# jscanvic/Scale-Equivariant-Imaging

Hardware: AMD Instinct MI355X
Metric: training images/sec (256x256 crops), proposed-loss deblur (higher is better)
Workload: dtype bf16; 1 GPU; BASELINE configs[1]: deblurring Gaussian_R2 noise=5, proposed loss (SURE + scale-EI), 256x256 pairs cropped to 48 in Loss.forward, ConvolutionalModel hidden=32 scales=5; parameters=645063043, batch_per_gpu=32, global_batch=32, parallelism=dp1

## Files before the change

include/sei_hip.h:

```cpp
#ifndef SEI_HIP_H
#define SEI_HIP_H

#include <stddef.h>
#include <stdint.h>

#ifdef __cplusplus
extern "C" {
#endif

#define SEI_OK 0
#define SEI_ERR_BAD_ARG 10001
#define SEI_ERR_TOO_LARGE 10002


#define SEI_ABI_VERSION 12
int sei_abi_version(void);
int sei_build_target(char *name, int n);

int sei_event_create(void **event);
int sei_event_destroy(void *event);
int sei_event_record_external(void *event, void *stream);
int sei_stream_wait_event(void *stream, void *event);

int sei_graph_node_counts(void *graph, int *kernel_nodes, int *all_nodes);
// ... 301 lines not shown
                         float *D32, uint16_t *D16, int M, int N, int epilogue, const float *bias, void *stream);
int sei_gemm_bf16nt_conv_unpad(const uint16_t *Ap, int cin_pad, const int *row_off9, const uint16_t *B, int ldb, float *y,
                               const float *res, int Bimg, int H, int W, int N, const float *bias, int act, void *stream);

int sei_adam_fused(float *param, const void *grad, int grad_is_bf16, float *exp_avg, float *exp_avg_sq,
                   size_t n, float lr, float beta1, float beta2, float eps, float weight_decay, int step,
                   float grad_scale, uint16_t *param_bf16, void *stream);

int sei_gemm_bf16nt_dw2_adam(const uint16_t *A1, const uint16_t *A2, int lda, const uint16_t *B1, const uint16_t *B2,
                             int ldb, float *param, float *exp_avg, float *exp_avg_sq, uint16_t *param_bf16,
                             const float *hyper, int M, int N, int K1, int K2, void *stream);
int sei_gemm_bf16nt_dw2_adam_ex(const uint16_t *A1, const uint16_t *A2, int lda, const uint16_t *B1, const uint16_t *B2,
                                int ldb, float *param, float *exp_avg, float *exp_avg_sq, uint16_t *param_bf16,
                                const float *hyper, int M, int N, int K1, int K2, int tile, void *stream);
size_t sei_gemm_bf16nt_dw2_adam_plan(int M, int N, int K1, int K2, int tile);
int sei_adam_scalars(float lr, float beta1, float beta2, float eps, float weight_decay, int step, float *out6_host,
                     void *stream);
int sei_adam_scalars_to_device(float lr, float beta1, float beta2, float eps, float weight_decay, int step,
                               float *dev6, void *stream);

size_t sei_sgd_partials(size_t lo, size_t hi, int grid_cap);
int sei_sgd_fused(float *param, const float *grad, const float *anchor, const float *coef64, size_t lo, size_t hi,
                  float lr, float grad_scale, uint16_t *param_bf16, double *partials, int grid_cap, void *stream);
int sei_sgd_penalty_finish(const double *partials, size_t count, float *penalty, void *stream);

size_t sei_adam_anchor_partials(size_t lo, size_t hi, int grid_cap);
int sei_adam_anchor_fused(float *param, const float *grad, float *exp_avg, float *exp_avg_sq, const float *anchor,
                          const float *coef64, size_t lo, size_t hi, float lr, float beta1, float beta2, float eps,
                          float weight_decay, int step, float grad_scale, uint16_t *param_bf16, double *partials,
                          int grid_cap, void *stream);
// ... 128 lines not shown
```

scale-equivariant-imaging_amd/_native.py:

```python
import ctypes
import os

import torch

_HERE = os.path.dirname(os.path.abspath(__file__))
LIB_PATH = os.environ.get("SEI_HIP_LIBRARY") or os.path.join(_HERE, "libsei_hip.so")

SEI_REDUCE_BLOCKS = 256

_c = ctypes
_P, _I, _F, _Z, _L = _c.c_void_p, _c.c_int, _c.c_float, _c.c_size_t, _c.c_longlong

SIGNATURES = {
    "sei_abi_version": [],
    "sei_event_create": [_P],
    "sei_event_destroy": [_P],
    "sei_event_record_external": [_P, _P],
    "sei_stream_wait_event": [_P, _P],
    "sei_graph_node_counts": [_P, _P, _P],
    "sei_build_target": [_c.c_char_p, _I],
    "sei_blur_sep_circ": [_P, _P, _P, _P, _I, _I, _I, _I, _I, _I, _P],
    "sei_blur_dense_circ": [_P, _P, _P, _I, _I, _I, _I, _I, _I, _P],
    "sei_blur_dense_pad": [_P, _P, _P, _I, _I, _I, _I, _I, _I, _I, _P, _P],
    "sei_circ_filter_sep": [_P, _P, _P, _P, _I, _I, _I, _P],
# ... 61 lines not shown
    "sei_gelu_f32": [_P, _P, _Z, _P],
    "sei_mul_dgelu_f32": [_P, _P, _Z, _P],
    "sei_cast_transpose_bf16": [_P, _I, _P, _P, _I, _I, _I, _P, _P],
    "sei_cast_bf16_colsum_weighted": [_P, _P, _P, _P, _I, _I, _P],
    "sei_cast_bf16_colsum_parts": [_P, _P, _P, _P, _I, _I, _P],
    "sei_gemm_bf16nt": [_P, _I, _I, _P, _I, _I, _P, _P, _I, _I, _I, _I, _P, _P, _P, _P, _P],
    "sei_gemm_bf16nt_colsum": [_P, _I, _I, _P, _I, _I, _P, _I, _I, _I, _I, _P, _P, _P],
    "sei_gemm_bf16nt_ws": [_P, _I, _I, _P, _I, _I, _P, _P, _I, _I, _I, _I, _P, _P, _P, _P, _P, _P, _Z, _I, _I, _I, _P],
    "sei_fold_many": [_P, _I, _P],
    "sei_transpose_bf16_many": [_P, _I, _P],
    "sei_gemm_bf16nt_dw2": [_P, _P, _I, _P, _P, _I, _P, _I, _I, _I, _I, _I, _P],
    "sei_gemm_bf16nt_ex": [_P, _I, _I, _P, _I, _I, _P, _P, _I, _I, _I, _I, _P, _P, _P, _P, _I, _I, _P],
    "sei_gemm_bf16nt_dw2_ex": [_P, _P, _I, _P, _P, _I, _P, _I, _I, _I, _I, _I, _I, _P],
    "sei_gemm_bf16nt_dw2_adam": [_P, _P, _I, _P, _P, _I, _P, _P, _P, _P, _P, _I, _I, _I, _I, _P],
    "sei_gemm_bf16nt_dw2_adam_ex": [_P, _P, _I, _P, _P, _I, _P, _P, _P, _P, _P, _I, _I, _I, _I, _I, _P],
    "sei_gemm_bf16nt_dw2_bf16out": [_P, _P, _I, _P, _P, _I, _P, _I, _I, _I, _I, _P],
    "sei_gemm_bf16nt_dw2_taps": [_P, _P, _I, _P, _P, _I, _P, _I, _I, _I, _I, _I, _I, _P, _L, _P],
    "sei_sepmap2": [_P, _P, _I, _I, _I, _I, _I, _I, _P, _P, _P, _P, _P, _Z, _P],
    "sei_sepmap2_big_pack": [_P, _P, _P, _P, _P, _I, _I, _I, _I, _P],
    "sei_sepmap2_big": [_P, _P, _I, _I, _I, _I, _I, _I, _P, _P, _P],
    "sei_sepmap2_packed": [_P, _P, _I, _I, _I, _I, _I, _I, _P, _P, _P, _Z, _P],
    "sei_sepmap2_bf16": [_P, _P, _I, _I, _I, _I, _I, _I, _P, _P],
    "sei_sepmap2_bf16_pack": [_P, _P, _P, _P, _P, _I, _I, _I, _I, _P],
    "sei_sepmap2_small": [_P, _P, _I, _I, _I, _I, _I, _I, _I, _P, _P, _P, _P, _P],
    "sei_sepmap2_bf16_out16": [_P, _P, _I, _I, _I, _I, _I, _I, _P, _P],
    "sei_colsum_f32": [_P, _P, _Z, _I, _P],
    "sei_colsum_weighted_f32": [_P, _P, _P, _Z, _I, _P],
    "sei_mlp_fused_fwd": [_P, _P, _P, _P, _P, _P, _F, _P, _I, _I, _P],
    "sei_mlp_fused_bwd": [_P, _P, _P, _P, _P, _P, _P, _P, _P, _P, _I, _I, _P],
    "sei_swin_attn_fwd": [_P, _P, _P, _I, _I, _I, _I, _I, _I, _F, _P],
# ... 62 lines not shown
    _fields_ = [("Y1", _P), ("Y2", _P), ("X1", _P), ("X2", _P), ("ldy", _I), ("ldx", _I), ("y0", _I), ("x0", _I),
                ("D", _P), ("ldd", _I)]


TOKGRAD_MAX_BLOCKS = 16


class DwStreamJob(_c.Structure):
    _fields_ = [("Y1", _P), ("Y2", _P), ("X1", _P), ("X2", _P), ("ldy", _I), ("ldx", _I), ("Mo", _I), ("Ni", _I),
                ("D", _P), ("ldd", _I), ("reserved", _I), ("K1", _L), ("K2", _L), ("gbias", _P)]


DWSTREAM_MAX_JOBS = 64


class FoldJob(_c.Structure):
    _fields_ = [("a", _P), ("b", _P), ("c", _P), ("ncol", _I), ("split", _I), ("kind", _I), ("nseg", _I),
                ("part", _P * 3), ("groups", _I * 3), ("reserved", _I)]


FOLD_SPLIT, FOLD_DWCONV7, FOLD_MAX_JOBS = 0, 1, 48


class TransposeJob(_c.Structure):
    _fields_ = [("src", _P), ("dst", _P), ("R", _I), ("C", _I)]


TRANSPOSE_MAX_JOBS = 16

CG_STATE_WORDS, CG_DONE, CG_ITERATIONS = 8, 3, 4
# ... 20 lines not shown
    "sei_sepmap2_big_work_elems": [_I, _I, _I, _I, _I, _I],
    "sei_swin_partials_floats": [_I],
    "sei_tokgrad_bf16_eligible": [_I, _I, _I, _I, _L, _L],
    "sei_dwstream_bf16_eligible": [_I, _I, _I, _I, _L, _L],
    "sei_mlp_fused_eligible": [_L, _I],
    "sei_rowgemm_bf16_eligible": [_L, _I, _I, _I, _I],
    "sei_rowgemm_lnbwd_bf16_eligible": [_L, _I, _I],
    "sei_rowgemm_lnbwd_work_floats": [_I],
    "sei_ln_bwd_part_offset": [_Z, _I],
    "sei_ln_bwd_part_count": [_Z, _I],
    "sei_rowgemm_dgelu_bf16_eligible": [_L, _I, _I],
    "sei_rowgemm_ln_bf16_eligible": [_L, _I, _I],
    "sei_gemm_bf16nt_plan": [_I, _I, _I, _I, _I, _I, _I, _I],
    "sei_gemm_bf16nt_plan_ws": [_I, _I, _I, _I, _I, _I, _I, _I, _Z],
    "sei_gemm_bf16nt_dw2_adam_plan": [_I, _I, _I, _I, _I],
    "sei_conv3x3_bwd_weight_parts_count": [_I, _I, _I, _I, _I, _I, _I],
    "sei_sepmap2_small_eligible": [_I, _I, _I, _I, _I, _I],
    "sei_cast_bf16_colsum_parts_count": [_I, _I],
    "sei_sgd_partials": [_Z, _Z, _I],
    "sei_adam_anchor_partials": [_Z, _Z, _I],
    "sei_drunet_work_bytes": [_I, _I, _I],
    "sei_cg_partials": [_Z],
    "sei_dps_partials": [_I, _Z],
    "sei_bm3d_ref_blocks": [_I, _I, _I],
    "sei_adm_gn_part_floats": [_I, _I],
}
ABI_VERSION = 12


class NativeLibraryError(RuntimeError):
# ... 33 lines not shown
    else:
        code = lib().sei_gemm_bf16nt_plan(int(a_rmajor), int(b_rmajor), int(out_f32), int(out_bf16), M, Nn, K, epilogue)
    if code == 0:
        raise NativeLibraryError("sei_gemm_bf16nt_plan: arguments sei_gemm_bf16nt would refuse")
    plan = {1: "nt", 2: "pq"}[code >> 48], (code >> 32) & 0xFFFF, (code >> 16) & 0xFFFF, code & 0x7FFF
    return plan + (bool(code & 0x8000),) if ws_bytes else plan


def adam_gemm_plan(M, Nn, K1, K2, tile=0):
    code = lib().sei_gemm_bf16nt_dw2_adam_plan(M, Nn, K1, K2, tile)
    if code == 0:
        raise NativeLibraryError("sei_gemm_bf16nt_dw2_adam_plan: arguments sei_gemm_bf16nt_dw2_adam_ex would refuse")
    return {1: "nt", 2: "pq"}[code >> 48], (code >> 32) & 0xFFFF, (code >> 16) & 0xFFFF, code & 0x7FFF


def stream():
    return torch.cuda.current_stream().cuda_stream


def check_tensor(t, name="tensor", dtype=torch.float32):
    if not isinstance(t, torch.Tensor):
        raise TypeError(f"{name}: expected a torch.Tensor, got {type(t).__name__}")
    if not t.is_cuda:
        raise NativeLibraryError(
            f"{name} is on {t.device}: this build runs on MI355X only (HIP kernels, no CPU path); "
            "use the CPU oracle under oracle/ for host-side checks")
    if t.dtype != dtype:
        raise TypeError(f"{name}: expected {dtype}, got {t.dtype}")
    if not t.is_contiguous():
        raise ValueError(f"{name}: expected a contiguous tensor")
# ... 93 lines not shown
```

scale-equivariant-imaging_amd/csrc/gemm_bf16nt.hip:

```cpp
#include "rm_image.h"

namespace {

constexpr int BK = 64;
constexpr int ROW_BYTES = 128;
constexpr int NWAVES = 8, NT = 512;

__device__ __attribute__((aligned(16))) unsigned short g_zero_chunk[8] = {0, 0, 0, 0, 0, 0, 0, 0};

struct NtArgs {
    const unsigned short *A = nullptr, *B = nullptr;
    float *D32 = nullptr;
    unsigned short *D16 = nullptr;
    int M = 0, N = 0, K = 0, lda = 0, ldb = 0;
    int epilogue = 0;
    const float *bias = nullptr, *R1 = nullptr, *R2 = nullptr;
    unsigned short *D2_16 = nullptr;
    int splitk = 1, k_per_split = 0;
    int tiles_m = 0, tiles_n = 0;
    int tiles_per_xcd = 0, band = 0;
    const unsigned short *A2 = nullptr, *B2 = nullptr;
    int k_seg = 0;
    int force_tile = 0, force_band = 0;
    float *colsum = nullptr;
    unsigned long long *plan = nullptr;
    int conv_cin = 0;
    int conv_off[9] = {};
    float *adam_p = nullptr, *adam_m = nullptr, *adam_v = nullptr;
    unsigned short *adam_p16 = nullptr;
    const float *adam_h = nullptr;
    int batch = 1;
    int batch_row[9] = {};
    long long batch_ld = 0;
    int unpad_H = 0, unpad_W = 0, unpad_act = 0;
    float *ws_slab = nullptr;
    unsigned *ws_cnt = nullptr;
    void *ws = nullptr;
    size_t ws_bytes = 0;
    int force_splitk = 0;
};

__device__ __forceinline__ float4 nt_load4(const float *p) {
    const f32x4 v = __builtin_nontemporal_load(reinterpret_cast<const f32x4 *>(p));
    return make_float4(v.x, v.y, v.z, v.w);
}
__device__ __forceinline__ void nt_store4(float *p, const float4 v) {
    f32x4 t;
    t.x = v.x; t.y = v.y; t.z = v.z; t.w = v.w;
    __builtin_nontemporal_store(t, reinterpret_cast<f32x4 *>(p));
}


template <int ROWS>
__device__ __forceinline__ void stage_piece(const unsigned short *__restrict__ G, int ld, int row0, int row_lim,
// ... 65 lines not shown
    static_assert(!BRM || BN % 128 == 0, "a reduction-major B tile is BN/128 images of 64 k-rows x 128 columns");
    constexpr int KS = stage_rows<TN, ARM, BRM, NSTAGE>();
    constexpr int A_BYTES = BM * ROW_BYTES * KS / BK;
    constexpr int IMG = 256 * KS;
    constexpr int STAGE = (BM + BN) * ROW_BYTES * KS / BK;
    __shared__ __attribute__((aligned(1024))) char smem[NSTAGE * STAGE];

    const int lane = threadIdx.x & 63;
    const int wave = __builtin_amdgcn_readfirstlane(threadIdx.x >> 6);
    const int wm = wave / WN, wn = wave % WN;
    const int li = lane & 31, lh = lane >> 5;

    int bid = blockIdx.x;
    const unsigned short *Bp = g.B, *B2p = g.B2;
    float *D32p = g.D32;
    if constexpr (ROWEPI == 3) {
        const int per = gridDim.x / g.batch, bt = bid / per;
        bid -= bt * per;
        const ptrdiff_t shift = (ptrdiff_t)g.batch_row[bt] * g.ldb;
        Bp += shift;
        B2p += shift;
        D32p += (size_t)bt * g.batch_ld;
    }
    int zs, ord;
    if (g.tiles_per_xcd == 0) {
        const int ntile = g.tiles_m * g.tiles_n;
        zs = bid / ntile;
        ord = bid - zs * ntile;
    } else {
        const int per_split = 8 * g.tiles_per_xcd;
        zs = bid / per_split;
        bid -= zs * per_split;
        ord = (bid & 7) * g.tiles_per_xcd + (bid >> 3);
        if ((bid >> 3) >= g.tiles_per_xcd || ord >= g.tiles_m * g.tiles_n) return;
    }
    int tm_i, tn_i;
    {
        const int band_tiles = g.tiles_m * g.band;
        const int b = ord / band_tiles, r = ord - b * band_tiles;
        const int width = min(g.band, g.tiles_n - b * g.band);
        tm_i = r / width;
        tn_i = b * g.band + (r - tm_i * width);
    }
    const int m0 = tm_i * BM, n0 = tn_i * BN;
    const int M = g.M, N = g.N, K = g.K;
    const int k_begin = zs * g.k_per_split;
    const int k_end = min(K, k_begin + g.k_per_split);

    f32x16 acc[TM][TN];
#pragma unroll
    for (int i = 0; i < TM; ++i)
#pragma unroll
        for (int j = 0; j < TN; ++j)
#pragma unroll
            for (int r = 0; r < 16; ++r) acc[i][j][r] = 0.f;

    constexpr bool PREFETCH_AUX = false;
    const int epi = g.epilogue;
    const bool lead = zs == 0;
    const bool split = g.splitk > 1;
    const float *aux1p = nullptr, *aux2p = nullptr;
    if (epi == SEI_EPI_BIAS_RES && (!split || lead)) { aux1p = g.R1; aux2p = g.R2; }
// ... 25 lines not shown
#pragma unroll
                for (int j = 0; j < TN; ++j)
#pragma unroll
                    for (int r = 0; r < 16; ++r) a1[i][j][r] = a2[i][j][r] = 0.f;
        }
    }

    constexpr int NPA = ARM ? 2 * KS / BK : (BM + 63) / 64, NPB = (BN / 64) * KS / BK;
    static_assert(BN % 64 == 0, "whole pieces per wave");
    unsigned off_a[NPA], off_b[NPB];
#pragma unroll
    for (int e = 0; e < NPA; ++e) {
        const int q = wave + NWAVES * e;
        if constexpr (ARM) {
            const int row = 4 * q + (lane >> 4), ch = (lane & 15) ^ swz_rmajor(row);
            off_a[e] = (unsigned)row * (unsigned)g.lda * 2u + 2u * (unsigned)min(8 * ch, M - 8 - m0);
        } else {
            const int row = 8 * q + (lane >> 3), c = (lane & 7) ^ ((row >> 1) & 7);
            off_a[e] = (unsigned)min(row, M - 1 - m0) * (unsigned)g.lda * 2u + 16u * c;
        }
    }
#pragma unroll
    for (int e = 0; e < NPB; ++e) {
        const int q = wave + NWAVES * e;
        if constexpr (BRM) {
            constexpr int PPI = KS / 4;
            const int im = q / PPI, qq = q % PPI;
            const int row = 4 * qq + (lane >> 4), ch = (lane & 15) ^ swz_rmajor(row);
            off_b[e] = (unsigned)row * (unsigned)g.ldb * 2u +
                       2u * (unsigned)max(min(128 * im + 8 * ch, N - 8 - n0), 0);
        } else {
            const int row = 8 * q + (lane >> 3), c = (lane & 7) ^ ((row >> 1) & 7);
            off_b[e] = (unsigned)min(row, N - 1 - n0) * (unsigned)g.ldb * 2u + 16u * c;
        }
    }
    auto rm_base = [&](const unsigned short *X1, const unsigned short *X2, int ld, int o0, int k0) -> const char * {
        if (k0 + KS <= g.k_seg && k0 + KS <= k_end) return reinterpret_cast<const char *>(X1 + (size_t)k0 * ld + o0);
        if (k0 >= g.k_seg && k0 + KS <= k_end) return reinterpret_cast<const char *>(X2 + (size_t)(k0 - g.k_seg) * ld + o0);
        return nullptr;
    };
    auto stage = [&](int k0, char *dst) {
        const char *ab, *bb;
        if constexpr (ARM) ab = rm_base(g.A, g.A2, g.lda, m0, k0);
        else if (g.conv_cin > 0) {
            const int tap = k0 / g.conv_cin;
            ab = reinterpret_cast<const char *>(g.A + ((ptrdiff_t)m0 + g.conv_off[tap]) * (ptrdiff_t)g.lda +
                                                (k0 - tap * g.conv_cin));
        }
        else ab = k0 + BK <= k_end ? reinterpret_cast<const char *>(g.A + (size_t)m0 * g.lda + k0) : nullptr;
        if (ab) {
#pragma unroll
            for (int e = 0; e < NPA; ++e)
                if (ARM || wave + NWAVES * e < BM / 8)
                    dma16_base(ab, off_a[e], dst + (wave + NWAVES * e) * 1024);
        } else {
            if constexpr (ARM) stage_tile_rmajor<KS>(g.A, g.A2, g.k_seg, g.lda, m0, M, k0, k_end, dst, wave, lane);
            else stage_tile<BM>(g.A, g.lda, m0, M, k0, k_end, dst, wave, lane);
        }
        if constexpr (BRM) bb = rm_base(Bp, B2p, g.ldb, n0, k0);
        else bb = k0 + BK <= k_end ? reinterpret_cast<const char *>(Bp + (size_t)n0 * g.ldb + k0) : nullptr;
        if (bb) {
#pragma unroll
            for (int e = 0; e < NPB; ++e)
                dma16_base(bb, off_b[e], dst + A_BYTES + (wave + NWAVES * e) * 1024);
        } else if constexpr (BRM) {
#pragma unroll
            for (int im = 0; im < BN / 128; ++im)
                stage_tile_rmajor<KS>(Bp, B2p, g.k_seg, g.ldb, n0 + 128 * im, N, k0, k_end,
                                      dst + A_BYTES + im * IMG, wave, lane);
        } else {
            stage_tile<BN>(Bp, g.ldb, n0, N, k0, k_end, dst + A_BYTES, wave, lane);
        }
    };
    const int sw = (li >> 1) & 7;
    const int a_off = (wm * 32 * TM + li) * ROW_BYTES;
    const int b_off = A_BYTES + (wn * 32 * TN + li) * ROW_BYTES;

    auto compute = [&](const char *now) {
#pragma unroll
        for (int s = 0; s < KS / 16; ++s) {
            const int pc = ((2 * s + lh) ^ sw) * 16;
            bf16x8 a[TM], b[TN];
#pragma unroll
// ... 77 lines not shown
            __syncthreads();
#pragma unroll
            for (int k = 0; k < 4; ++k) {
                const int idx = threadIdx.x + NT * k, r = idx >> 5, c4 = idx & 31;
                const int row = m0 + 64 * h + r, col = n0 + 4 * c4;
                if (row >= M || col >= N) continue;
                const float4 v = *reinterpret_cast<const float4 *>(patch + r * 128 + 4 * c4);
                uint2 w;
                w.x = sei_pack2_bf16(v.x, v.y);
                w.y = sei_pack2_bf16(v.z, v.w);
                *reinterpret_cast<uint2 *>(g.D16 + (size_t)row * N + col) = w;
            }
        }
        return;
    }
    if constexpr (ROWEPI == 1) {
        static_assert(TM == 2 && (TN == 1 || TN == 2) && WM == 2 && WN == 4, "the row patch below is laid out for 128-row tiles");
        static_assert(64 * BN * 4 <= NSTAGE * STAGE, "half a tile of float32 fits the operand stages");
        constexpr int QSH = TN == 1 ? 5 : 6;
        const float beta1 = g.adam_h[0], beta2 = g.adam_h[1], eps = g.adam_h[2], wd = g.adam_h[3];
        const float step_size = g.adam_h[4], inv_bc2_sqrt = g.adam_h[5];
        float *patch = reinterpret_cast<float *>(smem);
#pragma unroll
        for (int h = 0; h < 2; ++h) {
            __builtin_amdgcn_s_barrier();
            if constexpr (TN == 2) {
#pragma unroll
                for (int j = 0; j < TN; ++j)
#pragma unroll
                    for (int r = 0; r < 16; ++r)
                        patch[(32 * wm + 4 * lh + (r & 3) + 8 * (r >> 2)) * BN + 32 * TN * wn + 32 * j + li] = acc[h][j][r];
// ... 5 lines not shown
                        patch[(32 * i + 4 * lh + (r & 3) + 8 * (r >> 2)) * 128 + 32 * wn + li] = acc[i][0][r];
            }
            __syncthreads();
#pragma unroll 1
          for (int kk = 0; kk < 64 * BN / (4 * NT); kk += 2) {
            float4 gq[2], pq[2], mq[2], vq[2];
            size_t off[2];
            bool ok[2];
#pragma unroll
            for (int k = 0; k < 2; ++k) {
                const int idx = threadIdx.x + NT * (kk + k), r = idx >> QSH, c4 = idx & (BN / 4 - 1);
                const int row = m0 + (TN == 2 ? 64 * (r >> 5) + 32 * h + (r & 31) : 64 * h + r), col = n0 + 4 * c4;
                ok[k] = row < M && col < N;
                off[k] = ok[k] ? (size_t)row * N + col : 0;
                gq[k] = *reinterpret_cast<const float4 *>(patch + r * BN + 4 * c4);
                pq[k] = nt_load4(g.adam_p + off[k]);
                mq[k] = nt_load4(g.adam_m + off[k]);
                vq[k] = nt_load4(g.adam_v + off[k]);
            }
#pragma unroll
            for (int k = 0; k < 2; ++k) {
                if (!ok[k]) continue;
                float4 o;
                o.x = sei_adam_element(pq[k].x, gq[k].x, mq[k].x, vq[k].x, beta1, beta2, eps, wd, step_size, inv_bc2_sqrt);
                o.y = sei_adam_element(pq[k].y, gq[k].y, mq[k].y, vq[k].y, beta1, beta2, eps, wd, step_size, inv_bc2_sqrt);
                o.z = sei_adam_element(pq[k].z, gq[k].z, mq[k].z, vq[k].z, beta1, beta2, eps, wd, step_size, inv_bc2_sqrt);
                o.w = sei_adam_element(pq[k].w, gq[k].w, mq[k].w, vq[k].w, beta1, beta2, eps, wd, step_size, inv_bc2_sqrt);
                nt_store4(g.adam_m + off[k], mq[k]);
                nt_store4(g.adam_v + off[k], vq[k]);
                nt_store4(g.adam_p + off[k], o);
                if (g.adam_p16) {
                    uint2 w;
                    w.x = sei_pack2_bf16(o.x, o.y);
                    w.y = sei_pack2_bf16(o.z, o.w);
                    u32x2 t;
                    t.x = w.x; t.y = w.y;
                    __builtin_nontemporal_store(t, reinterpret_cast<u32x2 *>(g.adam_p16 + off[k]));
                }
            }
          }
        }
        return;
    }

    if constexpr ((ROWEPI == 4 || ROWEPI == 5) && patch_fits<TM, TN, WM, WN, NSTAGE>()) {
        constexpr int ROWS_WM = 32 * TM;
        constexpr int LDS_ROWS = (NSTAGE * STAGE) / (BN * 4);
        constexpr int GW = LDS_ROWS >= WM * ROWS_WM ? WM : (LDS_ROWS >= 2 * ROWS_WM && WM >= 2 ? 2 : 1);
        static_assert(LDS_ROWS >= ROWS_WM && WM % GW == 0, "one wave row of the tile fits the operand stages");
        constexpr int RP = GW * ROWS_WM, QPR = BN / 4, TOTAL = RP * QPR;
        float *patch = reinterpret_cast<float *>(smem);
        const bool to_bf16_only = g.D16 != nullptr && D32p == nullptr;
// ... 124 lines not shown
                    atomicAdd(D32p + o, v + a1[i][j][r] + a2[i][j][r]);
                    continue;
                }
                if (epi == SEI_EPI_MUL_DGELU)
                    v *= (g.D16 && !D32p) ? sei_dgelu_bf16out(a1[i][j][r]) : sei_dgelu(a1[i][j][r]);
                else if (epi == SEI_EPI_BIAS_SCALE_RES) v = fmaf(v, g.R1[row], a1[i][j][r]);
                else v += a1[i][j][r] + a2[i][j][r];
                if (epi == SEI_EPI_BIAS_GELU) g.D2_16[o] = sei_f2bf(sei_gelu_bf16out(v));
                if (D32p) D32p[o] = v;
                if (g.D16) g.D16[o] = sei_f2bf(v);
            }
        }
    }
}

__global__ __launch_bounds__(256) void zero_fill_kernel(float *__restrict__ p, size_t n) {
    const size_t stride = (size_t)gridDim.x * blockDim.x;
    const size_t n4 = n / 4;
    for (size_t i = (size_t)blockIdx.x * blockDim.x + threadIdx.x; i < n4; i += stride)
        reinterpret_cast<float4 *>(p)[i] = make_float4(0.f, 0.f, 0.f, 0.f);
    for (size_t i = n4 * 4 + (size_t)blockIdx.x * blockDim.x + threadIdx.x; i < n; i += stride) p[i] = 0.f;
}

#ifdef SEI_TUNING
int g_tuning_tile = 0, g_tuning_band = 0, g_tuning_splitk = 0;
#include "gemm_bf16pp.h"
#endif
#include "gemm_bf16pq.h"

template <int TM, int TN, int WM, int WN, bool ARM = false, bool BRM = false, int NSTAGE = 2, int ROWEPI = 0>
// ... 153 lines not shown
    }
    g.force_splitk = best_sk;
    return 10 * rf + best_nf;
}

int pq_choose_rr(const NtArgs &g) {
    if (g.force_tile != 0 || g.K < 2048 || g.M % 256 != 0 || g.N % 256 != 0 || !pq_eligible(g, true)) return 0;
    const size_t t4 = (size_t)(g.M / 256) * (size_t)(g.N / 256);
    if (t4 < 192 || (double)t4 / (double)(sei_ceil_div(t4, 256) * 256) < 0.8) return 0;
    return 84;
}

bool pq_adam_auto(const NtArgs &) { return false; }

bool adam_wide_fits(const NtArgs &g) { return g.M % 128 == 0 && g.N % 256 == 0; }
bool adam_wide_auto(const NtArgs &g) {
    if (!adam_wide_fits(g)) return false;
    const size_t tiles = (size_t)(g.M / 128) * (size_t)(g.N / 256);
    if (tiles < 512 || (double)tiles / (double)(sei_ceil_div(tiles, 512) * 512) < 0.8) return false;
    return g.K >= 2048 || tiles >= 4096;
}
constexpr int ADAM_WIDE_BAND = 8;

extern "C" int sei_colsum_bf16(const uint16_t *X, float *out, size_t M, int N, void *stream);

namespace {

int nt_fill_plain(NtArgs &g, const uint16_t *A, int lda, const uint16_t *B, int ldb, int M, int N, int K) {
    SEI_REQUIRE(A && B && M > 0 && N > 0 && K > 0);
    g.A = A; g.B = B; g.M = M; g.N = N; g.K = K; g.lda = lda; g.ldb = ldb;
    g.A2 = A; g.B2 = B; g.k_seg = K;
    return SEI_OK;
}

int nt_fill_dw2(NtArgs &g, const uint16_t *A1, const uint16_t *A2, int lda, const uint16_t *B1, const uint16_t *B2, int ldb,
// ... 303 lines not shown
    if (nt_fill_dw2(g, fake16, fake16, M, fake16, fake16, N, M, N, K1, K2, 1) != SEI_OK) return 0;
    g.D32 = fake32;
    g.adam_p = g.adam_m = g.adam_v = fake32; g.adam_h = fake32;
    g.plan = &plan;
    return dw2_adam_dispatch(g, tile, nullptr) == SEI_OK ? (size_t)plan : 0;
}

extern "C" int sei_gemm_bf16nt_dw2_adam(const uint16_t *A1, const uint16_t *A2, int lda, const uint16_t *B1,
                                        const uint16_t *B2, int ldb, float *param, float *exp_avg, float *exp_avg_sq,
                                        uint16_t *param_bf16, const float *hyper, int M, int N, int K1, int K2,
                                        void *stream) {
    return sei_gemm_bf16nt_dw2_adam_ex(A1, A2, lda, B1, B2, ldb, param, exp_avg, exp_avg_sq, param_bf16, hyper, M, N, K1, K2,
                                       0, stream);
}

extern "C" int sei_gemm_bf16nt_dw2_bf16out(const uint16_t *A1, const uint16_t *A2, int lda, const uint16_t *B1,
                                           const uint16_t *B2, int ldb, uint16_t *D16, int M, int N, int K1, int K2,
                                           void *stream) {
    NtArgs g;
    SEI_REQUIRE(D16 && ((uintptr_t)D16 & 7) == 0 && nt_fill_dw2(g, A1, A2, lda, B1, B2, ldb, M, N, K1, K2, 1) == SEI_OK);
    g.D16 = D16;
    if (K1 + K2 <= 1024) return launch_nt<2, 1, 2, 4, true, true, 1, 2>(g, (hipStream_t)stream);
    return launch_nt<2, 1, 2, 4, true, true, 2, 2>(g, (hipStream_t)stream);
}

extern "C" int sei_gemm_bf16nt_dw2_taps(const uint16_t *A1, const uint16_t *A2, int lda, const uint16_t *B1,
                                        const uint16_t *B2, int ldb, float *D32, int M, int N, int K1, int K2,
                                        int accumulate, int ntaps, const int *tap_rows, long long tap_ld, void *stream) {
    NtArgs g;
    SEI_REQUIRE(D32 && tap_rows && nt_fill_dw2(g, A1, A2, lda, B1, B2, ldb, M, N, K1, K2, 0) == SEI_OK);
// ... 57 lines not shown
```

scale-equivariant-imaging_amd/models/_wgrad.py:

```python
import collections
import os
import weakref

import torch

import _native as N
from . import _gemm
from ._gemm import EPI_ACCUM, EPI_NONE, _gemm_call, gemm_mixed, gemm_nt16

TOKEN_STREAMING = os.environ.get("SEI_SWIN_TILED") != "1"

DWSTREAM = os.environ.get("SEI_NO_DWSTREAM") != "1"

DEFERRED_FOLDS = os.environ.get("SEI_NO_DEFERRED_FOLDS") != "1"

SINK_ADAM, SINK_BF16 = "adam", "direct16"
_SINKS = {SINK_ADAM: ("sei_gemm_bf16nt_dw2_adam", "fused optimizer step"),
          SINK_BF16: ("sei_gemm_bf16nt_dw2_bf16out", "bf16 gradients written into the exchange buffer")}

_Queued = collections.namedtuple("_Queued", "job operands grad flops")


def _segments(pairs):
    (g1, x1), (g2, x2) = pairs[0], pairs[-1]
    return g1, x1, g2, x2, g1.shape[0], (g2.shape[0] if len(pairs) == 2 else 0)


def colsum16_into(acc, x16):
    M, Nn = x16.shape
    N.call("sei_colsum_bf16", x16.data_ptr(), acc.data_ptr(), M, Nn)


def _dwstream_ok(grad2d, pairs):
    if not DWSTREAM or not grad2d.is_cuda or grad2d.dim() != 2 or grad2d.dtype != torch.float32 or len(pairs) > 2 \
            or grad2d.stride(1) != 1:
# ... 12 lines not shown
                 "sink_launched")

    def __init__(self, ident):
        self.ident = ident
        self.arrivals, self.written = 0, False
        self.bias = None
        self.numel = self.flops_per_row = None
        self.taps = None
        self.whole_step = False
        self.sink, self.sink_launched = None, False


class WeightGradState:

    __slots__ = ("uses", "records", "parked", "store", "store_min", "merge", "flush_queued", "milestone", "milestone_done",
                 "dwjobs", "folds", "__weakref__")

    def __init__(self):
        self.uses = 0
        self.records = {}
        self.parked = {}
        self.store, self.store_min = False, 0
        self.merge = True
        self.flush_queued = False
        self.milestone, self.milestone_done = None, False
        self.dwjobs = []
        self.folds = {}

    def record(self, key, shape, tapped=False):
        rec = self.records.get(key)
        if rec is None or rec.ident != (tuple(shape), tapped):
            rec = self.records[key] = GradRecord((tuple(shape), tapped))
        return rec

    def meet(self, grad, flops_per_row=None, taps=None):
        rec = self.record(grad.data_ptr(), grad.shape, taps is not None)
        rec.numel, rec.flops_per_row, rec.taps = grad.numel(), flops_per_row, taps
        return rec

    def set_sinks(self, kind, table):
        for rec in self.records.values():
            if rec.sink is not None and rec.sink[0] == kind:
                rec.sink, rec.sink_launched = None, False
        for key, views in (table or {}).items():
            rec = self.record(key, views[0].shape)
            rec.sink, rec.sink_launched = (kind, views), False

    def sink_launches(self, kind):
        return {k for k, r in self.records.items() if r.sink_launched and r.sink[0] == kind}

    def arrive(self, pkey, n, entry, launch):
        partner = self.parked.pop(pkey, None)
        if partner is not None:
            launch([partner, entry])
        elif self.merge and n < self.uses and self.queue_flush():
            self.parked[pkey] = entry
        else:
            launch([entry])
# ... 23 lines not shown
        bias, rec.bias = rec.bias, None
        if bias is not None and (store or not _dwstream_ok(grad2d, pairs)):
            for gy16, _ in pairs:
                colsum16_into(bias, gy16)
            bias = None
        Np, Kp = grad2d.shape[-2:]
        g1, x1, g2, x2, K1, K2 = _segments(pairs)
        operands = (g1.data_ptr(), g2.data_ptr(), Np, x1.data_ptr(), x2.data_ptr(), Kp)
        if rec.sink is not None:
            kind, views = rec.sink
            entry, what = _SINKS[kind]
            if not (store and rec.whole_step) or rec.sink_launched:
                raise RuntimeError(f"{what}: a registered weight did not receive its gradient as one merged storing GEMM "
                                   "(different loss / batch / call count than planned)")
            rec.sink_launched = True
            _gemm_call(2.0 * Np * Kp * (K1 + K2), entry, *operands, *[N.ptr(v) for v in views], Np, Kp, K1, K2)
            return
        taps = rec.taps
        if taps is not None:
            T = grad2d.shape[0]
            per_row = rec.flops_per_row or 2.0 * T * Np * Kp
            if (K1 + K2) % 8 != 0:
                raise ValueError("weight_grad16 with taps: the reduction length must be a multiple of 8 rows")
            if TOKEN_STREAMING and not store and Np == 192 and Kp == 192 and T <= N.TOKGRAD_MAX_BLOCKS \
                    and K1 % 64 == 0 and K2 % 64 == 0 \
                    and g1.stride(0) == Np and x1.stride(0) == Kp and grad2d.is_contiguous():
                blocks = [N.TokGradBlock(g1.data_ptr(), g2.data_ptr(), x1.data_ptr() + 2 * Kp * int(taps[t]),
                                         x2.data_ptr() + 2 * Kp * int(taps[t]), Np, Kp, 0, 0,
                                         grad2d.data_ptr() + 4 * t * Np * Kp, Kp) for t in range(T)]
                arr = (N.TokGradBlock * T)(*blocks)
                _gemm_call(per_row * (K1 + K2), "sei_tokgrad_bf16_blocks", arr, T, K1, K2)
# ... 69 lines not shown
        g1, x1, g2, x2, K1, K2 = _segments(pairs)
        job = N.DwStreamJob(g1.data_ptr(), g2.data_ptr(), x1.data_ptr(), x2.data_ptr(), Np, Kp, Np, Kp, grad2d.data_ptr(),
                            grad2d.stride(0), 0, K1, K2, N.ptr(bias))
        self.dwjobs.append(_Queued(job, (g1, x1, g2, x2, bias), grad2d, per_row * (K1 + K2)))
        if len(self.dwjobs) == N.DWSTREAM_MAX_JOBS or not self.queue_flush():
            self.flush_dwstream()
        return True

    def flush_dwstream(self):
        jobs, self.dwjobs = self.dwjobs, []
        if not jobs:
            return
        arr = (N.DwStreamJob * len(jobs))(*[q.job for q in jobs])
        _gemm_call(sum(q.flops for q in jobs), "sei_dwstream_bf16_jobs", arr, len(jobs))

    def defer_fold(self, a, b, c, ncol, split, kind, work, offset, groups):
        if not self.queue_flush():
            return False
        key = a.data_ptr()
        meta = (N.ptr(b), N.ptr(c), int(ncol), int(split), int(kind))
        job = self.folds.get(key)
        if job is not None and (job["meta"] != meta or len(job["segs"]) == 3):
            self.flush_folds()
            job = None
        if job is None:
            if len(self.folds) == N.FOLD_MAX_JOBS:
                self.flush_folds()
            job = self.folds[key] = {"meta": meta, "segs": []}
        job["segs"].append((work, work.data_ptr() + 4 * int(offset), int(groups)))
        return True
# ... 17 lines not shown
                torch.autograd.Variable._execution_engine.queue_callback(self.flush)
            except RuntimeError:
                return False
            self.flush_queued = True
        return True

    def flush(self):
        self.flush_queued = False
        parked, self.parked = self.parked, {}
        for entry in parked.values():
            if isinstance(entry, list):
                self.launch_group([entry])
            else:
                self.launch(entry[2], [entry[:2]])
        self.flush_dwstream()
        self.flush_folds()


_DEFAULT_STATE = WeightGradState()
_RANGES = []


def state_of(owner=None):
    if owner is None:
        return _DEFAULT_STATE
    st = owner.__dict__.get("_sei_dw_state")
    if st is None:
        st = owner.__dict__["_sei_dw_state"] = WeightGradState()
    return st

# ... 106 lines not shown
```

Baseline: 2796 images/s.

## Batch fused weight-gradient Adam GEMMs into one grouped kernel launch

Adds a grouped variant of the fused dW GEMM plus Adam kernel. Up to eight per-weight jobs are packed into one launch, and each block looks up its job from cumulative tile offsets. The Python weight-grad state now queues eligible Adam-sink GEMMs (mid-sized shapes below the many-rounds tile threshold) and flushes them together at the end of backward. This cuts launch count and fills the GPU better for small GEMMs, at the cost of delaying the optimizer work until the flush and adding per-block job-selection overhead.

```diff
diff --git a/include/sei_hip.h b/include/sei_hip.h
--- a/include/sei_hip.h
+++ b/include/sei_hip.h
@@ -339,6 +339,16 @@
                                 int ldb, float *param, float *exp_avg, float *exp_avg_sq, uint16_t *param_bf16,
                                 const float *hyper, int M, int N, int K1, int K2, int tile, void *stream);
 size_t sei_gemm_bf16nt_dw2_adam_plan(int M, int N, int K1, int K2, int tile);
+#define SEI_ADAM_GROUP_MAX_JOBS 8
+typedef struct SeiAdamGemmJob {
+    const uint16_t *A1, *A2;
+    const uint16_t *B1, *B2;
+    float *param, *exp_avg, *exp_avg_sq;
+    uint16_t *param_bf16;
+    int lda, ldb, M, N, K1, K2;
+} SeiAdamGemmJob;
+int sei_gemm_bf16nt_dw2_adam_group(const SeiAdamGemmJob *jobs, int njobs, const float *hyper, void *stream);
+size_t sei_gemm_bf16nt_dw2_adam_groupable(int M, int N, int K1, int K2);
 int sei_adam_scalars(float lr, float beta1, float beta2, float eps, float weight_decay, int step, float *out6_host,
                      void *stream);
 int sei_adam_scalars_to_device(float lr, float beta1, float beta2, float eps, float weight_decay, int step,
diff --git a/scale-equivariant-imaging_amd/_native.py b/scale-equivariant-imaging_amd/_native.py
--- a/scale-equivariant-imaging_amd/_native.py
+++ b/scale-equivariant-imaging_amd/_native.py
@@ -99,6 +99,7 @@
     "sei_gemm_bf16nt_dw2_ex": [_P, _P, _I, _P, _P, _I, _P, _I, _I, _I, _I, _I, _I, _P],
     "sei_gemm_bf16nt_dw2_adam": [_P, _P, _I, _P, _P, _I, _P, _P, _P, _P, _P, _I, _I, _I, _I, _P],
     "sei_gemm_bf16nt_dw2_adam_ex": [_P, _P, _I, _P, _P, _I, _P, _P, _P, _P, _P, _I, _I, _I, _I, _I, _P],
+    "sei_gemm_bf16nt_dw2_adam_group": [_P, _I, _P, _P],
     "sei_gemm_bf16nt_dw2_bf16out": [_P, _P, _I, _P, _P, _I, _P, _I, _I, _I, _I, _P],
     "sei_gemm_bf16nt_dw2_taps": [_P, _P, _I, _P, _P, _I, _P, _I, _I, _I, _I, _I, _I, _P, _L, _P],
     "sei_sepmap2": [_P, _P, _I, _I, _I, _I, _I, _I, _P, _P, _P, _P, _P, _Z, _P],
@@ -191,6 +192,14 @@
 DWSTREAM_MAX_JOBS = 64
 
 
+class AdamGemmJob(_c.Structure):
+    _fields_ = [("A1", _P), ("A2", _P), ("B1", _P), ("B2", _P), ("param", _P), ("exp_avg", _P), ("exp_avg_sq", _P),
+                ("param_bf16", _P), ("lda", _I), ("ldb", _I), ("M", _I), ("N", _I), ("K1", _I), ("K2", _I)]
+
+
+ADAM_GROUP_MAX_JOBS = 8
+
+
 class FoldJob(_c.Structure):
     _fields_ = [("a", _P), ("b", _P), ("c", _P), ("ncol", _I), ("split", _I), ("kind", _I), ("nseg", _I),
                 ("part", _P * 3), ("groups", _I * 3), ("reserved", _I)]
@@ -241,6 +250,7 @@
     "sei_gemm_bf16nt_plan": [_I, _I, _I, _I, _I, _I, _I, _I],
     "sei_gemm_bf16nt_plan_ws": [_I, _I, _I, _I, _I, _I, _I, _I, _Z],
     "sei_gemm_bf16nt_dw2_adam_plan": [_I, _I, _I, _I, _I],
+    "sei_gemm_bf16nt_dw2_adam_groupable": [_I, _I, _I, _I],
     "sei_conv3x3_bwd_weight_parts_count": [_I, _I, _I, _I, _I, _I, _I],
     "sei_sepmap2_small_eligible": [_I, _I, _I, _I, _I, _I],
     "sei_cast_bf16_colsum_parts_count": [_I, _I],
@@ -304,6 +314,10 @@
     return {1: "nt", 2: "pq"}[code >> 48], (code >> 32) & 0xFFFF, (code >> 16) & 0xFFFF, code & 0x7FFF
 
 
+def adam_gemm_groupable(M, Nn, K1, K2):
+    return lib().sei_gemm_bf16nt_dw2_adam_groupable(M, Nn, K1, K2) != 0
+
+
 def stream():
     return torch.cuda.current_stream().cuda_stream
 
diff --git a/scale-equivariant-imaging_amd/csrc/gemm_bf16nt.hip b/scale-equivariant-imaging_amd/csrc/gemm_bf16nt.hip
--- a/scale-equivariant-imaging_amd/csrc/gemm_bf16nt.hip
+++ b/scale-equivariant-imaging_amd/csrc/gemm_bf16nt.hip
@@ -1,3 +1,4 @@
+#include <climits>
 #include "rm_image.h"
 
 namespace {
@@ -38,6 +39,8 @@
     void *ws = nullptr;
     size_t ws_bytes = 0;
     int force_splitk = 0;
+    int job_end[SEI_ADAM_GROUP_MAX_JOBS] = {};
+    SeiAdamGemmJob jobs[SEI_ADAM_GROUP_MAX_JOBS] = {};
 };
 
 __device__ __forceinline__ float4 nt_load4(const float *p) {
@@ -133,6 +136,33 @@
     int bid = blockIdx.x;
     const unsigned short *Bp = g.B, *B2p = g.B2;
     float *D32p = g.D32;
+#define JOB_OR(local, field) (ROWEPI == 6 ? (local) : (g.field))
+#define J_TM JOB_OR(jtm, tiles_m)
+#define J_TN JOB_OR(jtn, tiles_n)
+#define J_TPX JOB_OR(jtpx, tiles_per_xcd)
+#define J_BAND JOB_OR(jband, band)
+#define J_LDA JOB_OR(jlda, lda)
+#define J_LDB JOB_OR(jldb, ldb)
+#define J_KSEG JOB_OR(jkseg, k_seg)
+#define J_A JOB_OR(jA, A)
+#define J_A2 JOB_OR(jA2, A2)
+    const unsigned short *jA = nullptr, *jA2 = nullptr;
+    float *jp = nullptr, *jm = nullptr, *jv = nullptr;
+    unsigned short *jp16 = nullptr;
+    int jM = 0, jN = 0, jK = 0, jlda = 0, jldb = 0, jkseg = 0, jtm = 0, jtn = 0, jtpx = 0, jband = 0;
+    if constexpr (ROWEPI == 6) {
+        int j = 0;
+#pragma unroll
+        for (int t = 0; t < SEI_ADAM_GROUP_MAX_JOBS - 1; ++t) j += bid >= g.job_end[t] ? 1 : 0;
+        if (j > 0) bid -= g.job_end[j - 1];
+        const SeiAdamGemmJob &jb = g.jobs[j];
+        jA = jb.A1; jA2 = jb.A2; Bp = jb.B1; B2p = jb.B2;
+        jp = jb.param; jm = jb.exp_avg; jv = jb.exp_avg_sq; jp16 = jb.param_bf16;
+        jM = jb.M; jN = jb.N; jK = jb.K1 + jb.K2; jlda = jb.lda; jldb = jb.ldb; jkseg = jb.K1;
+        jtm = jM / (32 * TM * WM); jtn = jN / (32 * TN * WN);
+        jband = min(g.band, jtn);
+        jtpx = jtm * jtn < 64 ? 0 : (jtm * jtn + 7) >> 3;
+    }
     if constexpr (ROWEPI == 3) {
         const int per = gridDim.x / g.batch, bt = bid / per;
         bid -= bt * per;
@@ -142,29 +172,31 @@
         D32p += (size_t)bt * g.batch_ld;
     }
     int zs, ord;
-    if (g.tiles_per_xcd == 0) {
-        const int ntile = g.tiles_m * g.tiles_n;
+    if (J_TPX == 0) {
+        const int ntile = J_TM * J_TN;
         zs = bid / ntile;
         ord = bid - zs * ntile;
+        if constexpr (ROWEPI == 6)
+            if (zs > 0) return;
     } else {
-        const int per_split = 8 * g.tiles_per_xcd;
+        const int per_split = 8 * J_TPX;
         zs = bid / per_split;
         bid -= zs * per_split;
-        ord = (bid & 7) * g.tiles_per_xcd + (bid >> 3);
-        if ((bid >> 3) >= g.tiles_per_xcd || ord >= g.tiles_m * g.tiles_n) return;
+        ord = (bid & 7) * J_TPX + (bid >> 3);
+        if ((bid >> 3) >= J_TPX || ord >= J_TM * J_TN) return;
     }
     int tm_i, tn_i;
     {
-        const int band_tiles = g.tiles_m * g.band;
+        const int band_tiles = J_TM * J_BAND;
         const int b = ord / band_tiles, r = ord - b * band_tiles;
-        const int width = min(g.band, g.tiles_n - b * g.band);
+        const int width = min(J_BAND, J_TN - b * J_BAND);
         tm_i = r / width;
-        tn_i = b * g.band + (r - tm_i * width);
+        tn_i = b * J_BAND + (r - tm_i * width);
     }
     const int m0 = tm_i * BM, n0 = tn_i * BN;
-    const int M = g.M, N = g.N, K = g.K;
-    const int k_begin = zs * g.k_per_split;
-    const int k_end = min(K, k_begin + g.k_per_split);
+    const int M = JOB_OR(jM, M), N = JOB_OR(jN, N), K = JOB_OR(jK, K);
+    const int k_begin = zs * JOB_OR(jK, k_per_split);
+    const int k_end = min(K, k_begin + JOB_OR(jK, k_per_split));
 
     f32x16 acc[TM][TN];
 #pragma unroll
@@ -220,10 +252,10 @@
         const int q = wave + NWAVES * e;
         if constexpr (ARM) {
             const int row = 4 * q + (lane >> 4), ch = (lane & 15) ^ swz_rmajor(row);
-            off_a[e] = (unsigned)row * (unsigned)g.lda * 2u + 2u * (unsigned)min(8 * ch, M - 8 - m0);
+            off_a[e] = (unsigned)row * (unsigned)J_LDA * 2u + 2u * (unsigned)min(8 * ch, M - 8 - m0);
         } else {
             const int row = 8 * q + (lane >> 3), c = (lane & 7) ^ ((row >> 1) & 7);
-            off_a[e] = (unsigned)min(row, M - 1 - m0) * (unsigned)g.lda * 2u + 16u * c;
+            off_a[e] = (unsigned)min(row, M - 1 - m0) * (unsigned)J_LDA * 2u + 16u * c;
         }
     }
 #pragma unroll
@@ -233,21 +265,21 @@
             constexpr int PPI = KS / 4;
             const int im = q / PPI, qq = q % PPI;
             const int row = 4 * qq + (lane >> 4), ch = (lane & 15) ^ swz_rmajor(row);
-            off_b[e] = (unsigned)row * (unsigned)g.ldb * 2u +
+            off_b[e] = (unsigned)row * (unsigned)J_LDB * 2u +
                        2u * (unsigned)max(min(128 * im + 8 * ch, N - 8 - n0), 0);
         } else {
             const int row = 8 * q + (lane >> 3), c = (lane & 7) ^ ((row >> 1) & 7);
-            off_b[e] = (unsigned)min(row, N - 1 - n0) * (unsigned)g.ldb * 2u + 16u * c;
+            off_b[e] = (unsigned)min(row, N - 1 - n0) * (unsigned)J_LDB * 2u + 16u * c;
         }
     }
     auto rm_base = [&](const unsigned short *X1, const unsigned short *X2, int ld, int o0, int k0) -> const char * {
-        if (k0 + KS <= g.k_seg && k0 + KS <= k_end) return reinterpret_cast<const char *>(X1 + (size_t)k0 * ld + o0);
-        if (k0 >= g.k_seg && k0 + KS <= k_end) return reinterpret_cast<const char *>(X2 + (size_t)(k0 - g.k_seg) * ld + o0);
+        if (k0 + KS <= J_KSEG && k0 + KS <= k_end) return reinterpret_cast<const char *>(X1 + (size_t)k0 * ld + o0);
+        if (k0 >= J_KSEG && k0 + KS <= k_end) return reinterpret_cast<const char *>(X2 + (size_t)(k0 - J_KSEG) * ld + o0);
         return nullptr;
     };
     auto stage = [&](int k0, char *dst) {
         const char *ab, *bb;
-        if constexpr (ARM) ab = rm_base(g.A, g.A2, g.lda, m0, k0);
+        if constexpr (ARM) ab = rm_base(J_A, J_A2, J_LDA, m0, k0);
         else if (g.conv_cin > 0) {
             const int tap = k0 / g.conv_cin;
             ab = reinterpret_cast<const char *>(g.A + ((ptrdiff_t)m0 + g.conv_off[tap]) * (ptrdiff_t)g.lda +
@@ -260,10 +292,10 @@
                 if (ARM || wave + NWAVES * e < BM / 8)
                     dma16_base(ab, off_a[e], dst + (wave + NWAVES * e) * 1024);
         } else {
-            if constexpr (ARM) stage_tile_rmajor<KS>(g.A, g.A2, g.k_seg, g.lda, m0, M, k0, k_end, dst, wave, lane);
+            if constexpr (ARM) stage_tile_rmajor<KS>(J_A, J_A2, J_KSEG, J_LDA, m0, M, k0, k_end, dst, wave, lane);
             else stage_tile<BM>(g.A, g.lda, m0, M, k0, k_end, dst, wave, lane);
         }
-        if constexpr (BRM) bb = rm_base(Bp, B2p, g.ldb, n0, k0);
+        if constexpr (BRM) bb = rm_base(Bp, B2p, J_LDB, n0, k0);
         else bb = k0 + BK <= k_end ? reinterpret_cast<const char *>(Bp + (size_t)n0 * g.ldb + k0) : nullptr;
         if (bb) {
 #pragma unroll
@@ -272,7 +304,7 @@
         } else if constexpr (BRM) {
 #pragma unroll
             for (int im = 0; im < BN / 128; ++im)
-                stage_tile_rmajor<KS>(Bp, B2p, g.k_seg, g.ldb, n0 + 128 * im, N, k0, k_end,
+                stage_tile_rmajor<KS>(Bp, B2p, J_KSEG, J_LDB, n0 + 128 * im, N, k0, k_end,
                                       dst + A_BYTES + im * IMG, wave, lane);
         } else {
             stage_tile<BN>(Bp, g.ldb, n0, N, k0, k_end, dst + A_BYTES, wave, lane);
@@ -380,7 +412,9 @@
         }
         return;
     }
-    if constexpr (ROWEPI == 1) {
+    if constexpr (ROWEPI == 1 || ROWEPI == 6) {
+        float *adam_p = JOB_OR(jp, adam_p), *adam_m = JOB_OR(jm, adam_m), *adam_v = JOB_OR(jv, adam_v);
+        unsigned short *adam_p16 = JOB_OR(jp16, adam_p16);
         static_assert(TM == 2 && (TN == 1 || TN == 2) && WM == 2 && WN == 4, "the row patch below is laid out for 128-row tiles");
         static_assert(64 * BN * 4 <= NSTAGE * STAGE, "half a tile of float32 fits the operand stages");
         constexpr int QSH = TN == 1 ? 5 : 6;
@@ -416,9 +450,9 @@
                 ok[k] = row < M && col < N;
                 off[k] = ok[k] ? (size_t)row * N + col : 0;
                 gq[k] = *reinterpret_cast<const float4 *>(patch + r * BN + 4 * c4);
-                pq[k] = nt_load4(g.adam_p + off[k]);
-                mq[k] = nt_load4(g.adam_m + off[k]);
-                vq[k] = nt_load4(g.adam_v + off[k]);
+                pq[k] = nt_load4(adam_p + off[k]);
+                mq[k] = nt_load4(adam_m + off[k]);
+                vq[k] = nt_load4(adam_v + off[k]);
             }
 #pragma unroll
             for (int k = 0; k < 2; ++k) {
@@ -428,16 +462,16 @@
                 o.y = sei_adam_element(pq[k].y, gq[k].y, mq[k].y, vq[k].y, beta1, beta2, eps, wd, step_size, inv_bc2_sqrt);
                 o.z = sei_adam_element(pq[k].z, gq[k].z, mq[k].z, vq[k].z, beta1, beta2, eps, wd, step_size, inv_bc2_sqrt);
                 o.w = sei_adam_element(pq[k].w, gq[k].w, mq[k].w, vq[k].w, beta1, beta2, eps, wd, step_size, inv_bc2_sqrt);
-                nt_store4(g.adam_m + off[k], mq[k]);
-                nt_store4(g.adam_v + off[k], vq[k]);
-                nt_store4(g.adam_p + off[k], o);
-                if (g.adam_p16) {
+                nt_store4(adam_m + off[k], mq[k]);
+                nt_store4(adam_v + off[k], vq[k]);
+                nt_store4(adam_p + off[k], o);
+                if (adam_p16) {
                     uint2 w;
                     w.x = sei_pack2_bf16(o.x, o.y);
                     w.y = sei_pack2_bf16(o.z, o.w);
                     u32x2 t;
                     t.x = w.x; t.y = w.y;
-                    __builtin_nontemporal_store(t, reinterpret_cast<u32x2 *>(g.adam_p16 + off[k]));
+                    __builtin_nontemporal_store(t, reinterpret_cast<u32x2 *>(adam_p16 + off[k]));
                 }
             }
           }
@@ -592,6 +626,16 @@
     }
 }
 
+#undef JOB_OR
+#undef J_TM
+#undef J_TN
+#undef J_TPX
+#undef J_BAND
+#undef J_LDA
+#undef J_LDB
+#undef J_KSEG
+#undef J_A
+#undef J_A2
 __global__ __launch_bounds__(256) void zero_fill_kernel(float *__restrict__ p, size_t n) {
     const size_t stride = (size_t)gridDim.x * blockDim.x;
     const size_t n4 = n / 4;
@@ -775,11 +819,15 @@
 bool pq_adam_auto(const NtArgs &) { return false; }
 
 bool adam_wide_fits(const NtArgs &g) { return g.M % 128 == 0 && g.N % 256 == 0; }
+constexpr size_t ADAM_WIDE_MANY_ROUNDS_TILES = 4096;
 bool adam_wide_auto(const NtArgs &g) {
     if (!adam_wide_fits(g)) return false;
     const size_t tiles = (size_t)(g.M / 128) * (size_t)(g.N / 256);
     if (tiles < 512 || (double)tiles / (double)(sei_ceil_div(tiles, 512) * 512) < 0.8) return false;
-    return g.K >= 2048 || tiles >= 4096;
+    return g.K >= 2048 || tiles >= ADAM_WIDE_MANY_ROUNDS_TILES;
+}
+bool adam_groupable(const NtArgs &g) {
+    return adam_wide_fits(g) && (size_t)(g.M / 128) * (size_t)(g.N / 256) < ADAM_WIDE_MANY_ROUNDS_TILES;
 }
 constexpr int ADAM_WIDE_BAND = 8;
 
@@ -1113,6 +1161,52 @@
                                        0, stream);
 }
 
+extern "C" int sei_gemm_bf16nt_dw2_adam_group(const SeiAdamGemmJob *jobs, int njobs, const float *hyper, void *stream) {
+    SEI_REQUIRE(jobs && hyper && njobs >= 1 && njobs <= SEI_ADAM_GROUP_MAX_JOBS);
+    NtArgs g;
+    struct Range { uintptr_t lo, hi; };
+    Range state[SEI_ADAM_GROUP_MAX_JOBS][4];
+    size_t blocks = 0;
+    for (int j = 0; j < njobs; ++j) {
+        const SeiAdamGemmJob &jb = jobs[j];
+        NtArgs one;
+        SEI_REQUIRE(jb.param && jb.exp_avg && jb.exp_avg_sq &&
+                    nt_fill_dw2(one, jb.A1, jb.A2, jb.lda, jb.B1, jb.B2, jb.ldb, jb.M, jb.N, jb.K1, jb.K2, 1) == SEI_OK);
+        SEI_REQUIRE((((uintptr_t)jb.param | (uintptr_t)jb.exp_avg | (uintptr_t)jb.exp_avg_sq) & 15) == 0 &&
+                    ((uintptr_t)jb.param_bf16 & 7) == 0);
+        SEI_REQUIRE(adam_wide_fits(one));
+        const size_t n = (size_t)jb.M * jb.N, tiles = (size_t)(jb.M / 128) * (size_t)(jb.N / 256);
+        SEI_REQUIRE(tiles < ((size_t)1 << 24));
+        const void *base[4] = {jb.param, jb.exp_avg, jb.exp_avg_sq, jb.param_bf16};
+        for (int a = 0; a < 4; ++a) {
+            const uintptr_t lo = (uintptr_t)base[a];
+            state[j][a] = {lo, base[a] ? lo + n * (a == 3 ? 2 : 4) : lo};
+            for (int i = 0; i < j; ++i)
+                for (int b = 0; b < 4; ++b)
+                    SEI_REQUIRE(!(state[j][a].lo < state[i][b].hi && state[i][b].lo < state[j][a].hi));
+        }
+        blocks += 8 * sei_ceil_div(tiles, 8);
+        g.jobs[j] = jb;
+        g.job_end[j] = (int)blocks;
+    }
+    for (int j = njobs; j < SEI_ADAM_GROUP_MAX_JOBS; ++j) g.job_end[j] = INT_MAX;
+    SEI_REQUIRE(blocks < ((size_t)1 << 27));
+    g.adam_h = hyper;
+    g.epilogue = SEI_EPI_NONE;
+    g.splitk = 1;
+    g.band = ADAM_WIDE_BAND;
+    hipLaunchKernelGGL((gemm_bf16nt_kernel<2, 2, 2, 4, true, true, 3, 6>), dim3((unsigned)blocks), dim3(NT), 0,
+                       (hipStream_t)stream, g);
+    return sei_launch_status();
+}
+
+extern "C" size_t sei_gemm_bf16nt_dw2_adam_groupable(int M, int N, int K1, int K2) {
+    const uint16_t *fake16 = reinterpret_cast<const uint16_t *>(uintptr_t(1) << 20);
+    NtArgs g;
+    if (nt_fill_dw2(g, fake16, fake16, M, fake16, fake16, N, M, N, K1, K2, 1) != SEI_OK) return 0;
+    return adam_groupable(g) ? 1 : 0;
+}
+
 extern "C" int sei_gemm_bf16nt_dw2_bf16out(const uint16_t *A1, const uint16_t *A2, int lda, const uint16_t *B1,
                                            const uint16_t *B2, int ldb, uint16_t *D16, int M, int N, int K1, int K2,
                                            void *stream) {
diff --git a/scale-equivariant-imaging_amd/models/_wgrad.py b/scale-equivariant-imaging_amd/models/_wgrad.py
--- a/scale-equivariant-imaging_amd/models/_wgrad.py
+++ b/scale-equivariant-imaging_amd/models/_wgrad.py
@@ -18,7 +18,10 @@
 _SINKS = {SINK_ADAM: ("sei_gemm_bf16nt_dw2_adam", "fused optimizer step"),
           SINK_BF16: ("sei_gemm_bf16nt_dw2_bf16out", "bf16 gradients written into the exchange buffer")}
 
+ADAM_GROUP = os.environ.get("SEI_NO_ADAM_GROUP") != "1"
+
 _Queued = collections.namedtuple("_Queued", "job operands grad flops")
+_QueuedAdam = collections.namedtuple("_QueuedAdam", "job operands hyper flops args")
 
 
 def _segments(pairs):
@@ -61,7 +64,7 @@
 class WeightGradState:
 
     __slots__ = ("uses", "records", "parked", "store", "store_min", "merge", "flush_queued", "milestone", "milestone_done",
-                 "dwjobs", "folds", "__weakref__")
+                 "dwjobs", "adamjobs", "folds", "__weakref__")
 
     def __init__(self):
         self.uses = 0
@@ -72,6 +75,7 @@
         self.flush_queued = False
         self.milestone, self.milestone_done = None, False
         self.dwjobs = []
+        self.adamjobs = []
         self.folds = {}
 
     def record(self, key, shape, tapped=False):
@@ -89,6 +93,8 @@
         for rec in self.records.values():
             if rec.sink is not None and rec.sink[0] == kind:
                 rec.sink, rec.sink_launched = None, False
+        if kind == SINK_ADAM:
+            self.adamjobs = []
         for key, views in (table or {}).items():
             rec = self.record(key, views[0].shape)
             rec.sink, rec.sink_launched = (kind, views), False
@@ -142,7 +148,9 @@
                 raise RuntimeError(f"{what}: a registered weight did not receive its gradient as one merged storing GEMM "
                                    "(different loss / batch / call count than planned)")
             rec.sink_launched = True
-            _gemm_call(2.0 * Np * Kp * (K1 + K2), entry, *operands, *[N.ptr(v) for v in views], Np, Kp, K1, K2)
+            args = (*operands, *[N.ptr(v) for v in views], Np, Kp, K1, K2)
+            if kind != SINK_ADAM or not self.queue_adam_group((g1, x1, g2, x2), views, args):
+                _gemm_call(2.0 * Np * Kp * (K1 + K2), entry, *args)
             return
         taps = rec.taps
         if taps is not None:
@@ -242,6 +250,31 @@
         arr = (N.DwStreamJob * len(jobs))(*[q.job for q in jobs])
         _gemm_call(sum(q.flops for q in jobs), "sei_dwstream_bf16_jobs", arr, len(jobs))
 
+    def queue_adam_group(self, operands, views, args):
+        Np, Kp, K1, K2 = args[-4:]
+        if not ADAM_GROUP or self.milestone is not None or not N.adam_gemm_groupable(Np, Kp, K1, K2):
+            return False
+        hyper = views[-1]
+        if self.adamjobs and self.adamjobs[0].hyper is not hyper:
+            self.flush_adam_group()
+        if not self.queue_flush():
+            return False
+        g1, x1, g2, x2 = operands
+        job = N.AdamGemmJob(g1.data_ptr(), g2.data_ptr(), x1.data_ptr(), x2.data_ptr(), *[N.ptr(v) for v in views[:4]],
+                            Np, Kp, Np, Kp, K1, K2)
+        self.adamjobs.append(_QueuedAdam(job, operands, hyper, 2.0 * Np * Kp * (K1 + K2), args))
+        return True
+
+    def flush_adam_group(self):
+        jobs, self.adamjobs = self.adamjobs, []
+        for i in range(0, len(jobs), N.ADAM_GROUP_MAX_JOBS):
+            chunk = jobs[i:i + N.ADAM_GROUP_MAX_JOBS]
+            if len(chunk) == 1:
+                _gemm_call(chunk[0].flops, _SINKS[SINK_ADAM][0], *chunk[0].args)
+                continue
+            arr = (N.AdamGemmJob * len(chunk))(*[q.job for q in chunk])
+            _gemm_call(sum(q.flops for q in chunk), "sei_gemm_bf16nt_dw2_adam_group", arr, len(chunk), N.ptr(chunk[0].hyper))
+
     def defer_fold(self, a, b, c, ncol, split, kind, work, offset, groups):
         if not self.queue_flush():
             return False
@@ -289,6 +322,7 @@
             else:
                 self.launch(entry[2], [entry[:2]])
         self.flush_dwstream()
+        self.flush_adam_group()
         self.flush_folds()
 
 
```

Result: faster. 2830 images/s, median of 6 (+1.2%).
